# saidwivedi/TokenHMR

Measured on NVIDIA H100. Metric: images/sec (256x192) at bs=64 per GPU, full TokenHMR forward, higher is better.
Workload: dtype f16 operands / f32 accumulate

## Files before the change

tokenhmr_b200/csrc/attention_mma.cuh:

```cuda
#pragma once
#include "common.cuh"
#include "ptx.cuh"

namespace thmr {

constexpr int kAttTokens = 192;
constexpr int kAttHeadDim = 80;
constexpr int kAttPitch = 88;
constexpr int kAttWarps = 6;
constexpr int kAttThreads = 32 * kAttWarps;
constexpr uint32_t kAttMatBytes = kAttTokens * kAttPitch * 2;
constexpr uint32_t kAttSmemBytes = 3 * kAttMatBytes;

struct AttnParams {
  const __half* qkv;
  int ldq;
  int num_problems;
  int heads;
  float scale_log2e;
  __half* out;
  int ldo;
  float* dbg_s;
  unsigned long long* stamp;
};

__device__ __forceinline__ float fast_exp2(float x) {
  float y;
  asm("ex2.approx.ftz.f32 %0, %1;" : "=f"(y) : "f"(x));
  return y;
}
__device__ __forceinline__ void ldmatrix_x4(uint32_t (&r)[4], uint32_t addr) {
  asm volatile("ldmatrix.sync.aligned.m8n8.x4.shared.b16 {%0, %1, %2, %3}, [%4];"
               : "=r"(r[0]), "=r"(r[1]), "=r"(r[2]), "=r"(r[3]) : "r"(addr));
}
__device__ __forceinline__ void ldmatrix_x4_trans(uint32_t (&r)[4], uint32_t addr) {
  asm volatile("ldmatrix.sync.aligned.m8n8.x4.trans.shared.b16 {%0, %1, %2, %3}, [%4];"
               : "=r"(r[0]), "=r"(r[1]), "=r"(r[2]), "=r"(r[3]) : "r"(addr));
}
__device__ __forceinline__ void mma_16816(float (&d)[4], const uint32_t (&a)[4], uint32_t b0, uint32_t b1) {
  asm volatile("mma.sync.aligned.m16n8k16.row.col.f32.f16.f16.f32 {%0, %1, %2, %3}, {%4, %5, %6, %7}, {%8, %9}, "
               "{%0, %1, %2, %3};"
               : "+f"(d[0]), "+f"(d[1]), "+f"(d[2]), "+f"(d[3])
               : "r"(a[0]), "r"(a[1]), "r"(a[2]), "r"(a[3]), "r"(b0), "r"(b1));
}
__device__ __forceinline__ uint32_t pack_half2(float a, float b) {
  __half2 h = __floats2half2_rn(a, b);
  return *reinterpret_cast<uint32_t*>(&h);
}

template <bool DBG>
__global__ void __launch_bounds__(kAttThreads, 2) vit_attention_kernel(const AttnParams p) {
  extern __shared__ __align__(16) uint8_t att_smem[];
  const uint32_t aQ = smem_u32(att_smem), aK = aQ + kAttMatBytes, aV = aK + kAttMatBytes;
  const int prob = blockIdx.x;
  const int b = prob / p.heads, h = prob % p.heads;
  const int warp = threadIdx.x >> 5, lane = threadIdx.x & 31;

  pdl_launch_dependents();
  stamp_start(p.stamp);
  pdl_wait();

  const __half* src = p.qkv + static_cast<size_t>(b) * kAttTokens * p.ldq;
  for (int i = threadIdx.x; i < 3 * kAttTokens * 10; i += kAttThreads) {
    const int m = i / (kAttTokens * 10), r = (i / 10) % kAttTokens, c = i % 10;
    const __half* g = src + static_cast<size_t>(r) * p.ldq + (m * p.heads + h) * kAttHeadDim + c * 8;
    const uint32_t s = aQ + m * kAttMatBytes + (r * kAttPitch + c * 8) * 2;
    asm volatile("cp.async.cg.shared.global [%0], [%1], 16;" ::"r"(s), "l"(g) : "memory");
  }
  asm volatile("cp.async.commit_group;\n\tcp.async.wait_group 0;" ::: "memory");
  __syncthreads();

  const int g = lane >> 2, t4 = lane & 3;
  for (int tile = warp; tile < kAttTokens / 16; tile += kAttWarps) {
    const int r0 = tile * 16;
    uint32_t qa[5][4];
#pragma unroll
    for (int kk = 0; kk < 5; ++kk)
      ldmatrix_x4(qa[kk], aQ + ((r0 + (lane & 15)) * kAttPitch + kk * 16 + 8 * (lane >> 4)) * 2);
    float s[24][4];
#pragma unroll
    for (int nt = 0; nt < 24; ++nt) s[nt][0] = s[nt][1] = s[nt][2] = s[nt][3] = 0.f;
#pragma unroll
    for (int np = 0; np < 12; ++np) {
#pragma unroll
      for (int kk = 0; kk < 5; ++kk) {
        uint32_t kb[4];
        ldmatrix_x4(kb, aK + ((np * 16 + (lane & 7) + 8 * (lane >> 4)) * kAttPitch + kk * 16 + 8 * ((lane >> 3) & 1)) * 2);
        mma_16816(s[2 * np], qa[kk], kb[0], kb[1]);
        mma_16816(s[2 * np + 1], qa[kk], kb[2], kb[3]);
      }
    }
    if (DBG) {
      float* d = p.dbg_s + (static_cast<size_t>(prob) * kAttTokens + r0 + g) * kAttTokens + 2 * t4;
#pragma unroll
      for (int nt = 0; nt < 24; ++nt) {
        *reinterpret_cast<float2*>(d + nt * 8) = make_float2(s[nt][0], s[nt][1]);
        *reinterpret_cast<float2*>(d + 8 * kAttTokens + nt * 8) = make_float2(s[nt][2], s[nt][3]);
      }
    }
    float mx0 = -INFINITY, mx1 = -INFINITY;
#pragma unroll
    for (int nt = 0; nt < 24; ++nt) {
      mx0 = fmaxf(mx0, fmaxf(s[nt][0], s[nt][1]));
      mx1 = fmaxf(mx1, fmaxf(s[nt][2], s[nt][3]));
    }
#pragma unroll
    for (int off = 1; off <= 2; off <<= 1) {
      mx0 = fmaxf(mx0, __shfl_xor_sync(0xffffffffu, mx0, off));
      mx1 = fmaxf(mx1, __shfl_xor_sync(0xffffffffu, mx1, off));
    }
    const float mo0 = mx0 * p.scale_log2e, mo1 = mx1 * p.scale_log2e;
    float sum0 = 0.f, sum1 = 0.f;
    uint32_t pa[12][4];
#pragma unroll
    for (int nt = 0; nt < 24; ++nt) {
      const float e0 = fast_exp2(fmaf(s[nt][0], p.scale_log2e, -mo0));
      const float e1 = fast_exp2(fmaf(s[nt][1], p.scale_log2e, -mo0));
      const float e2 = fast_exp2(fmaf(s[nt][2], p.scale_log2e, -mo1));
      const float e3 = fast_exp2(fmaf(s[nt][3], p.scale_log2e, -mo1));
      sum0 += e0 + e1;
      sum1 += e2 + e3;
      pa[nt >> 1][(nt & 1) * 2 + 0] = pack_half2(e0, e1);
      pa[nt >> 1][(nt & 1) * 2 + 1] = pack_half2(e2, e3);
    }
#pragma unroll
    for (int off = 1; off <= 2; off <<= 1) {
      sum0 += __shfl_xor_sync(0xffffffffu, sum0, off);
      sum1 += __shfl_xor_sync(0xffffffffu, sum1, off);
    }
    float o[10][4];
#pragma unroll
    for (int dt = 0; dt < 10; ++dt) o[dt][0] = o[dt][1] = o[dt][2] = o[dt][3] = 0.f;
#pragma unroll
    for (int ks = 0; ks < 12; ++ks) {
#pragma unroll
      for (int dp = 0; dp < 5; ++dp) {
        uint32_t vb[4];
        ldmatrix_x4_trans(vb, aV + ((ks * 16 + (lane & 7) + 8 * ((lane >> 3) & 1)) * kAttPitch + dp * 16 + 8 * (lane >> 4)) * 2);
        mma_16816(o[2 * dp], pa[ks], vb[0], vb[1]);
        mma_16816(o[2 * dp + 1], pa[ks], vb[2], vb[3]);
      }
    }
    const float inv0 = 1.0f / sum0, inv1 = 1.0f / sum1;
    __half* out = p.out + (static_cast<size_t>(b) * kAttTokens + r0 + g) * p.ldo + h * kAttHeadDim + 2 * t4;
#pragma unroll
    for (int dt = 0; dt < 10; ++dt) {
      *reinterpret_cast<uint32_t*>(out + dt * 8) = pack_half2(o[dt][0] * inv0, o[dt][1] * inv0);
      *reinterpret_cast<uint32_t*>(out + 8 * static_cast<size_t>(p.ldo) + dt * 8) = pack_half2(o[dt][2] * inv1, o[dt][3] * inv1);
    }
  }
}

struct AttnPlan {
  AttnParams p;
  int grid;
};

inline int attention_make_plan(const __half* qkv, int ld_qkv, int B, int heads, __half* out, int ldo, float* dbg_s,
                               AttnPlan* plan) {
  THMR_CHECK(B > 0 && heads > 0, "attention: bad shape");
  THMR_CHECK(ld_qkv >= 3 * heads * kAttHeadDim, "attention: qkv pitch %d < %d", ld_qkv, 3 * heads * kAttHeadDim);
  THMR_CHECK((reinterpret_cast<uintptr_t>(qkv) & 15) == 0 && ld_qkv % 8 == 0, "attention: qkv pointer/pitch alignment");
  THMR_CHECK(ldo % 2 == 0 && (reinterpret_cast<uintptr_t>(out) & 3) == 0, "attention: output alignment");
  plan->p.qkv = qkv;
  plan->p.ldq = ld_qkv;
  plan->p.num_problems = B * heads;
  plan->p.heads = heads;
  plan->p.scale_log2e = 1.4426950408889634f / sqrtf(static_cast<float>(kAttHeadDim));
  plan->p.out = out;
  plan->p.ldo = ldo;
  plan->p.dbg_s = dbg_s;
  plan->p.stamp = nullptr;
  plan->grid = plan->p.num_problems;
  return THMR_OK;
}

template <bool DBG>
inline int attention_launch_t(const AttnPlan& plan, cudaStream_t st) {
  static bool configured = false;
  if (!configured) {
    THMR_CUDA(cudaFuncSetAttribute(vit_attention_kernel<DBG>, cudaFuncAttributeMaxDynamicSharedMemorySize, kAttSmemBytes));
    configured = true;
  }
  THMR_CUDA(launch_pdl(vit_attention_kernel<DBG>, plan.grid, kAttThreads, kAttSmemBytes, st, plan.p));
  return THMR_OK;
}

inline int attention_dispatch(const AttnPlan& plan, cudaStream_t st) {
  return plan.p.dbg_s ? attention_launch_t<true>(plan, st) : attention_launch_t<false>(plan, st);
}

}
```

tokenhmr_b200/_build.py:

```python
from __future__ import annotations

import hashlib
import os
import subprocess
import sys
from pathlib import Path

PKG_DIR = Path(__file__).resolve().parent
CSRC = PKG_DIR / "csrc"
LIB_PATH = PKG_DIR / "libtokenhmr_b200.so"
STAMP = PKG_DIR / ".libtokenhmr_b200.stamp"
PROBE_SRC = PKG_DIR.parent / "tests" / "csrc" / "kernel_probe.cu"
PROBE_PATH = PKG_DIR.parent / "tests" / "libthmr_probe.so"
PROBE_STAMP = PKG_DIR.parent / "tests" / ".libthmr_probe.stamp"
GEMM_PROBE_SRC = PKG_DIR.parent / "tests" / "csrc" / "gemm_probe.cu"
GEMM_PROBE_PATH = PKG_DIR.parent / "tests" / "libthmr_gemm_probe.so"
GEMM_PROBE_STAMP = PKG_DIR.parent / "tests" / ".libthmr_gemm_probe.stamp"

NVCC_FLAGS = [
    "-gencode", "arch=compute_90a,code=sm_90a",
    "-lineinfo", "-O3", "-std=c++17",
    "--expt-relaxed-constexpr",
    "-Xcompiler", "-fPIC", "-shared",
]
PROBE_FLAGS = ["-Xcompiler", "-fvisibility=hidden"]


def _nvcc() -> str:
    for cand in (os.environ.get("NVCC"), "/usr/local/cuda/bin/nvcc", "nvcc"):
        if cand and (os.path.isabs(cand) and os.path.exists(cand) or not os.path.isabs(cand)):
            return cand
    return "nvcc"


def source_hash(probe: bool = False) -> str:
    h = hashlib.sha256()
    files = sorted(CSRC.glob("*.cu")) + sorted(CSRC.glob("*.cuh")) + sorted((PKG_DIR.parent / "include").glob("*.h"))
    if probe:
        files += sorted(PROBE_SRC.parent.glob("*.cu"))
    for f in files:
        h.update(f.name.encode())
        h.update(f.read_bytes())
    h.update(" ".join(NVCC_FLAGS + (PROBE_FLAGS if probe else [])).encode())
    return h.hexdigest()


def _compile(src: Path, out: Path, stamp: Path, flags: list, want: str, force: bool, verbose: bool) -> Path:
    if not force and out.exists() and stamp.exists() and stamp.read_text().strip() == want:
        return out
    cmd = [_nvcc(), *flags, "-o", str(out), str(src)]
    if verbose:
        cmd.insert(1, "-Xptxas=-v")
        print(" ".join(cmd), file=sys.stderr)
    res = subprocess.run(cmd, capture_output=True, text=True)
    if res.returncode != 0:
        raise RuntimeError(f"nvcc failed ({res.returncode}):\n{res.stdout}\n{res.stderr}")
    if verbose:
        print(res.stderr, file=sys.stderr)
    stamp.write_text(want)
    return out


def build_probe(force: bool = False, verbose: bool = False) -> Path:
    if GEMM_PROBE_SRC.exists():
        _compile(GEMM_PROBE_SRC, GEMM_PROBE_PATH, GEMM_PROBE_STAMP, NVCC_FLAGS + PROBE_FLAGS, source_hash(probe=True),
                 force, verbose)
    return _compile(PROBE_SRC, PROBE_PATH, PROBE_STAMP, NVCC_FLAGS + PROBE_FLAGS, source_hash(probe=True), force,
                    verbose)


def build(force: bool = False, verbose: bool = False) -> Path:
    path = _compile(CSRC / "tokenhmr_b200.cu", LIB_PATH, STAMP, NVCC_FLAGS, source_hash(), force, verbose)
    if PROBE_SRC.exists():
        build_probe(force, verbose)
    return path


if __name__ == "__main__":
    print(build(force="--force" in sys.argv, verbose="-v" in sys.argv))
```

tokenhmr_b200/csrc/ptx.cuh:

```cuda
#pragma once
#include <cuda.h>
#include <cuda_fp16.h>
#include <cuda_runtime.h>
#include <stdint.h>

namespace thmr {

__device__ unsigned int g_pipeline_timeout = 0;
constexpr uint32_t kSpinLimit = 1u << 24;

__device__ __forceinline__ uint32_t smem_u32(const void* p) {
  return static_cast<uint32_t>(__cvta_generic_to_shared(p));
}

__device__ __forceinline__ void sts_f32x2(uint32_t a, float x, float y) {
  asm volatile("st.shared.v2.f32 [%0], {%1, %2};" ::"r"(a), "f"(x), "f"(y));
}
__device__ __forceinline__ float4 lds_f32x4(uint32_t a) {
  float4 v;
  asm volatile("ld.shared.v4.f32 {%0, %1, %2, %3}, [%4];" : "=f"(v.x), "=f"(v.y), "=f"(v.z), "=f"(v.w) : "r"(a));
  return v;
}
__device__ __forceinline__ void sts_f32(uint32_t a, float x) { asm volatile("st.shared.f32 [%0], %1;" ::"r"(a), "f"(x)); }
__device__ __forceinline__ void sts_u32(uint32_t a, uint32_t x) { asm volatile("st.shared.b32 [%0], %1;" ::"r"(a), "r"(x)); }
// ... 70 lines not shown
  asm volatile("barrier.cluster.arrive.release;\n\tbarrier.cluster.wait.acquire;" ::: "memory");
}
__device__ __forceinline__ void mbar_arrive_cluster(uint64_t* bar, uint32_t cta) {
  asm volatile(
      "{\n\t"
      ".reg .b32 ra;\n\t"
      "mapa.shared::cluster.u32 ra, %0, %1;\n\t"
      "mbarrier.arrive.release.cluster.shared::cluster.b64 _, [ra];\n\t"
      "}\n" ::"r"(smem_u32(bar)),
      "r"(cta)
      : "memory");
}
__device__ __forceinline__ bool mbar_wait_cluster(uint64_t* bar, uint32_t parity) {
#pragma unroll 1
  for (uint32_t it = 0; it < kSpinLimit; ++it) {
    uint32_t ok;
    asm volatile(
        "{\n\t"
        ".reg .pred P;\n\t"
        "mbarrier.try_wait.parity.acquire.cluster.shared::cta.b64 P, [%1], %2;\n\t"
        "selp.u32 %0, 1, 0, P;\n\t"
        "}\n"
        : "=r"(ok)
        : "r"(smem_u32(bar)), "r"(parity)
        : "memory");
    if (ok) return true;
  }
  atomicExch(&g_pipeline_timeout, 1u);
  return false;
}

__device__ __forceinline__ void tma_prefetch_desc(const CUtensorMap* m) {
  asm volatile("prefetch.tensormap [%0];" ::"l"(reinterpret_cast<uint64_t>(m)) : "memory");
}
__device__ __forceinline__ void tma_load_2d(void* smem_dst, const CUtensorMap* m, uint64_t* bar, int32_t c0,
                                            int32_t c1) {
  asm volatile(
      "cp.async.bulk.tensor.2d.shared::cluster.global.mbarrier::complete_tx::bytes"
      " [%0], [%1, {%3, %4}], [%2];"
      :
      : "r"(smem_u32(smem_dst)), "l"(reinterpret_cast<uint64_t>(m)), "r"(smem_u32(bar)), "r"(c0), "r"(c1)
      : "memory");
}
__device__ __forceinline__ void tma_load_2d_mcast(void* smem_dst, const CUtensorMap* m, uint64_t* bar, int32_t c0,
                                                  int32_t c1, uint16_t cta_mask) {
  asm volatile(
      "cp.async.bulk.tensor.2d.shared::cluster.global.mbarrier::complete_tx::bytes.multicast::cluster"
      " [%0], [%1, {%3, %4}], [%2], %5;"
      :
      : "r"(smem_u32(smem_dst)), "l"(reinterpret_cast<uint64_t>(m)), "r"(smem_u32(bar)), "r"(c0), "r"(c1),
        "h"(cta_mask)
      : "memory");
}
__device__ __forceinline__ void tma_store_2d(const CUtensorMap* m, uint32_t smem_src, int32_t c0, int32_t c1) {
  asm volatile("cp.async.bulk.tensor.2d.global.shared::cta.bulk_group [%0, {%2, %3}], [%1];"
               :
               : "l"(reinterpret_cast<uint64_t>(m)), "r"(smem_src), "r"(c0), "r"(c1)
               : "memory");
}
__device__ __forceinline__ void tma_reduce_add_2d(const CUtensorMap* m, uint32_t smem_src, int32_t c0, int32_t c1) {
  asm volatile("cp.reduce.async.bulk.tensor.2d.global.shared::cta.add.tile.bulk_group [%0, {%2, %3}], [%1];"
               :
               : "l"(reinterpret_cast<uint64_t>(m)), "r"(smem_src), "r"(c0), "r"(c1)
               : "memory");
}
__device__ __forceinline__ void tma_store_commit() { asm volatile("cp.async.bulk.commit_group;" ::: "memory"); }
template <int N>
__device__ __forceinline__ void tma_store_wait_read() {
  asm volatile("cp.async.bulk.wait_group.read %0;" ::"n"(N) : "memory");
}
template <int N>
__device__ __forceinline__ void tma_store_wait() {
  asm volatile("cp.async.bulk.wait_group %0;" ::"n"(N) : "memory");
}

__device__ __forceinline__ uint64_t make_wgmma_desc_sw128(uint32_t saddr) {
  uint64_t d = 0;
  d |= static_cast<uint64_t>((saddr >> 4) & 0x3FFF);
  d |= static_cast<uint64_t>(1) << 16;
  d |= static_cast<uint64_t>(1024 >> 4) << 32;
  d |= static_cast<uint64_t>(1) << 62;
  return d;
}
__device__ __forceinline__ void wgmma_fence() { asm volatile("wgmma.fence.sync.aligned;" ::: "memory"); }
__device__ __forceinline__ void wgmma_commit() { asm volatile("wgmma.commit_group.sync.aligned;" ::: "memory"); }
template <int N>
__device__ __forceinline__ void wgmma_wait() {
  asm volatile("wgmma.wait_group.sync.aligned %0;" ::"n"(N) : "memory");
}
template <int N>
__device__ __forceinline__ void wgmma_fence_operand(float (&d)[N]) {
#pragma unroll
  for (int i = 0; i < N; ++i) asm volatile("" : "+f"(d[i])::"memory");
}

__device__ __forceinline__ void wgmma_m64n32k16(float (&d)[16], uint64_t da, uint64_t db, uint32_t scale_d) {
  asm volatile(
      "{\n\t.reg .pred p;\n\tsetp.ne.b32 p, %18, 0;\n\t"
      "wgmma.mma_async.sync.aligned.m64n32k16.f32.f16.f16 {%0, %1, %2, %3, %4, %5, %6, %7, %8, %9, %10, %11, %12, %13, %14, %15}, %16, %17, p, 1, 1, 0, 0;\n\t}\n"
      : "+f"(d[0]), "+f"(d[1]), "+f"(d[2]), "+f"(d[3]), "+f"(d[4]), "+f"(d[5]), "+f"(d[6]), "+f"(d[7]), "+f"(d[8]), "+f"(d[9]), "+f"(d[10]), "+f"(d[11]), "+f"(d[12]), "+f"(d[13]), "+f"(d[14]), "+f"(d[15])
      : "l"(da), "l"(db), "r"(scale_d));
}
__device__ __forceinline__ void wgmma_m64n64k16(float (&d)[32], uint64_t da, uint64_t db, uint32_t scale_d) {
  asm volatile(
      "{\n\t.reg .pred p;\n\tsetp.ne.b32 p, %34, 0;\n\t"
      "wgmma.mma_async.sync.aligned.m64n64k16.f32.f16.f16 {%0, %1, %2, %3, %4, %5, %6, %7, %8, %9, %10, %11, %12, %13, %14, %15, %16, %17, %18, %19, %20, %21, %22, %23, %24, %25, %26, %27, %28, %29, %30, %31}, %32, %33, p, 1, 1, 0, 0;\n\t}\n"
      : "+f"(d[0]), "+f"(d[1]), "+f"(d[2]), "+f"(d[3]), "+f"(d[4]), "+f"(d[5]), "+f"(d[6]), "+f"(d[7]), "+f"(d[8]), "+f"(d[9]), "+f"(d[10]), "+f"(d[11]), "+f"(d[12]), "+f"(d[13]), "+f"(d[14]), "+f"(d[15]), "+f"(d[16]), "+f"(d[17]), "+f"(d[18]), "+f"(d[19]), "+f"(d[20]), "+f"(d[21]), "+f"(d[22]), "+f"(d[23]), "+f"(d[24]), "+f"(d[25]), "+f"(d[26]), "+f"(d[27]), "+f"(d[28]), "+f"(d[29]), "+f"(d[30]), "+f"(d[31])
      : "l"(da), "l"(db), "r"(scale_d));
}
__device__ __forceinline__ void wgmma_m64n128k16(float (&d)[64], uint64_t da, uint64_t db, uint32_t scale_d) {
  asm volatile(
      "{\n\t.reg .pred p;\n\tsetp.ne.b32 p, %66, 0;\n\t"
      "wgmma.mma_async.sync.aligned.m64n128k16.f32.f16.f16 {%0, %1, %2, %3, %4, %5, %6, %7, %8, %9, %10, %11, %12, %13, %14, %15, %16, %17, %18, %19, %20, %21, %22, %23, %24, %25, %26, %27, %28, %29, %30, %31, %32, %33, %34, %35, %36, %37, %38, %39, %40, %41, %42, %43, %44, %45, %46, %47, %48, %49, %50, %51, %52, %53, %54, %55, %56, %57, %58, %59, %60, %61, %62, %63}, %64, %65, p, 1, 1, 0, 0;\n\t}\n"
      : "+f"(d[0]), "+f"(d[1]), "+f"(d[2]), "+f"(d[3]), "+f"(d[4]), "+f"(d[5]), "+f"(d[6]), "+f"(d[7]), "+f"(d[8]), "+f"(d[9]), "+f"(d[10]), "+f"(d[11]), "+f"(d[12]), "+f"(d[13]), "+f"(d[14]), "+f"(d[15]), "+f"(d[16]), "+f"(d[17]), "+f"(d[18]), "+f"(d[19]), "+f"(d[20]), "+f"(d[21]), "+f"(d[22]), "+f"(d[23]), "+f"(d[24]), "+f"(d[25]), "+f"(d[26]), "+f"(d[27]), "+f"(d[28]), "+f"(d[29]), "+f"(d[30]), "+f"(d[31]), "+f"(d[32]), "+f"(d[33]), "+f"(d[34]), "+f"(d[35]), "+f"(d[36]), "+f"(d[37]), "+f"(d[38]), "+f"(d[39]), "+f"(d[40]), "+f"(d[41]), "+f"(d[42]), "+f"(d[43]), "+f"(d[44]), "+f"(d[45]), "+f"(d[46]), "+f"(d[47]), "+f"(d[48]), "+f"(d[49]), "+f"(d[50]), "+f"(d[51]), "+f"(d[52]), "+f"(d[53]), "+f"(d[54]), "+f"(d[55]), "+f"(d[56]), "+f"(d[57]), "+f"(d[58]), "+f"(d[59]), "+f"(d[60]), "+f"(d[61]), "+f"(d[62]), "+f"(d[63])
      : "l"(da), "l"(db), "r"(scale_d));
}
__device__ __forceinline__ void wgmma_m64n256k16(float (&d)[128], uint64_t da, uint64_t db, uint32_t scale_d) {
  asm volatile(
      "{\n\t.reg .pred p;\n\tsetp.ne.b32 p, %130, 0;\n\t"
      "wgmma.mma_async.sync.aligned.m64n256k16.f32.f16.f16 {%0, %1, %2, %3, %4, %5, %6, %7, %8, %9, %10, %11, %12, %13, %14, %15, %16, %17, %18, %19, %20, %21, %22, %23, %24, %25, %26, %27, %28, %29, %30, %31, %32, %33, %34, %35, %36, %37, %38, %39, %40, %41, %42, %43, %44, %45, %46, %47, %48, %49, %50, %51, %52, %53, %54, %55, %56, %57, %58, %59, %60, %61, %62, %63, %64, %65, %66, %67, %68, %69, %70, %71, %72, %73, %74, %75, %76, %77, %78, %79, %80, %81, %82, %83, %84, %85, %86, %87, %88, %89, %90, %91, %92, %93, %94, %95, %96, %97, %98, %99, %100, %101, %102, %103, %104, %105, %106, %107, %108, %109, %110, %111, %112, %113, %114, %115, %116, %117, %118, %119, %120, %121, %122, %123, %124, %125, %126, %127}, %128, %129, p, 1, 1, 0, 0;\n\t}\n"
      : "+f"(d[0]), "+f"(d[1]), "+f"(d[2]), "+f"(d[3]), "+f"(d[4]), "+f"(d[5]), "+f"(d[6]), "+f"(d[7]), "+f"(d[8]), "+f"(d[9]), "+f"(d[10]), "+f"(d[11]), "+f"(d[12]), "+f"(d[13]), "+f"(d[14]), "+f"(d[15]), "+f"(d[16]), "+f"(d[17]), "+f"(d[18]), "+f"(d[19]), "+f"(d[20]), "+f"(d[21]), "+f"(d[22]), "+f"(d[23]), "+f"(d[24]), "+f"(d[25]), "+f"(d[26]), "+f"(d[27]), "+f"(d[28]), "+f"(d[29]), "+f"(d[30]), "+f"(d[31]), "+f"(d[32]), "+f"(d[33]), "+f"(d[34]), "+f"(d[35]), "+f"(d[36]), "+f"(d[37]), "+f"(d[38]), "+f"(d[39]), "+f"(d[40]), "+f"(d[41]), "+f"(d[42]), "+f"(d[43]), "+f"(d[44]), "+f"(d[45]), "+f"(d[46]), "+f"(d[47]), "+f"(d[48]), "+f"(d[49]), "+f"(d[50]), "+f"(d[51]), "+f"(d[52]), "+f"(d[53]), "+f"(d[54]), "+f"(d[55]), "+f"(d[56]), "+f"(d[57]), "+f"(d[58]), "+f"(d[59]), "+f"(d[60]), "+f"(d[61]), "+f"(d[62]), "+f"(d[63]), "+f"(d[64]), "+f"(d[65]), "+f"(d[66]), "+f"(d[67]), "+f"(d[68]), "+f"(d[69]), "+f"(d[70]), "+f"(d[71]), "+f"(d[72]), "+f"(d[73]), "+f"(d[74]), "+f"(d[75]), "+f"(d[76]), "+f"(d[77]), "+f"(d[78]), "+f"(d[79]), "+f"(d[80]), "+f"(d[81]), "+f"(d[82]), "+f"(d[83]), "+f"(d[84]), "+f"(d[85]), "+f"(d[86]), "+f"(d[87]), "+f"(d[88]), "+f"(d[89]), "+f"(d[90]), "+f"(d[91]), "+f"(d[92]), "+f"(d[93]), "+f"(d[94]), "+f"(d[95]), "+f"(d[96]), "+f"(d[97]), "+f"(d[98]), "+f"(d[99]), "+f"(d[100]), "+f"(d[101]), "+f"(d[102]), "+f"(d[103]), "+f"(d[104]), "+f"(d[105]), "+f"(d[106]), "+f"(d[107]), "+f"(d[108]), "+f"(d[109]), "+f"(d[110]), "+f"(d[111]), "+f"(d[112]), "+f"(d[113]), "+f"(d[114]), "+f"(d[115]), "+f"(d[116]), "+f"(d[117]), "+f"(d[118]), "+f"(d[119]), "+f"(d[120]), "+f"(d[121]), "+f"(d[122]), "+f"(d[123]), "+f"(d[124]), "+f"(d[125]), "+f"(d[126]), "+f"(d[127])
      : "l"(da), "l"(db), "r"(scale_d));
}

__device__ __forceinline__ void wgmma_m64n64k32_e4m3(float (&d)[32], uint64_t da, uint64_t db, uint32_t scale_d) {
  asm volatile(
      "{\n\t.reg .pred p;\n\tsetp.ne.b32 p, %34, 0;\n\t"
      "wgmma.mma_async.sync.aligned.m64n64k32.f32.e4m3.e4m3 {%0, %1, %2, %3, %4, %5, %6, %7, %8, %9, %10, %11, %12, %13, %14, %15, %16, %17, %18, %19, %20, %21, %22, %23, %24, %25, %26, %27, %28, %29, %30, %31}, %32, %33, p, 1, 1;\n\t}\n"
      : "+f"(d[0]), "+f"(d[1]), "+f"(d[2]), "+f"(d[3]), "+f"(d[4]), "+f"(d[5]), "+f"(d[6]), "+f"(d[7]), "+f"(d[8]), "+f"(d[9]), "+f"(d[10]), "+f"(d[11]), "+f"(d[12]), "+f"(d[13]), "+f"(d[14]), "+f"(d[15]), "+f"(d[16]), "+f"(d[17]), "+f"(d[18]), "+f"(d[19]), "+f"(d[20]), "+f"(d[21]), "+f"(d[22]), "+f"(d[23]), "+f"(d[24]), "+f"(d[25]), "+f"(d[26]), "+f"(d[27]), "+f"(d[28]), "+f"(d[29]), "+f"(d[30]), "+f"(d[31])
      : "l"(da), "l"(db), "r"(scale_d));
}
__device__ __forceinline__ void wgmma_m64n128k32_e4m3(float (&d)[64], uint64_t da, uint64_t db, uint32_t scale_d) {
  asm volatile(
      "{\n\t.reg .pred p;\n\tsetp.ne.b32 p, %66, 0;\n\t"
      "wgmma.mma_async.sync.aligned.m64n128k32.f32.e4m3.e4m3 {%0, %1, %2, %3, %4, %5, %6, %7, %8, %9, %10, %11, %12, %13, %14, %15, %16, %17, %18, %19, %20, %21, %22, %23, %24, %25, %26, %27, %28, %29, %30, %31, %32, %33, %34, %35, %36, %37, %38, %39, %40, %41, %42, %43, %44, %45, %46, %47, %48, %49, %50, %51, %52, %53, %54, %55, %56, %57, %58, %59, %60, %61, %62, %63}, %64, %65, p, 1, 1;\n\t}\n"
      : "+f"(d[0]), "+f"(d[1]), "+f"(d[2]), "+f"(d[3]), "+f"(d[4]), "+f"(d[5]), "+f"(d[6]), "+f"(d[7]), "+f"(d[8]), "+f"(d[9]), "+f"(d[10]), "+f"(d[11]), "+f"(d[12]), "+f"(d[13]), "+f"(d[14]), "+f"(d[15]), "+f"(d[16]), "+f"(d[17]), "+f"(d[18]), "+f"(d[19]), "+f"(d[20]), "+f"(d[21]), "+f"(d[22]), "+f"(d[23]), "+f"(d[24]), "+f"(d[25]), "+f"(d[26]), "+f"(d[27]), "+f"(d[28]), "+f"(d[29]), "+f"(d[30]), "+f"(d[31]), "+f"(d[32]), "+f"(d[33]), "+f"(d[34]), "+f"(d[35]), "+f"(d[36]), "+f"(d[37]), "+f"(d[38]), "+f"(d[39]), "+f"(d[40]), "+f"(d[41]), "+f"(d[42]), "+f"(d[43]), "+f"(d[44]), "+f"(d[45]), "+f"(d[46]), "+f"(d[47]), "+f"(d[48]), "+f"(d[49]), "+f"(d[50]), "+f"(d[51]), "+f"(d[52]), "+f"(d[53]), "+f"(d[54]), "+f"(d[55]), "+f"(d[56]), "+f"(d[57]), "+f"(d[58]), "+f"(d[59]), "+f"(d[60]), "+f"(d[61]), "+f"(d[62]), "+f"(d[63])
      : "l"(da), "l"(db), "r"(scale_d));
}

__device__ __forceinline__ uint16_t cvt_e4m3x2(float lo, float hi) {
  uint16_t r;
  asm("cvt.rn.satfinite.e4m3x2.f32 %0, %1, %2;" : "=h"(r) : "f"(hi), "f"(lo));
  return r;
}

__device__ __forceinline__ float e4m3_scale(float amax) {
  if (!(amax > 0.f)) return 1.0f;
  int E;
  const float m = frexpf(amax, &E);
  return ldexpf(1.0f, m <= 0.875f ? E - 9 : E - 8);
}

__device__ __forceinline__ void bulk_load_1d(void* smem_dst, const void* src, uint32_t bytes, uint64_t* bar) {
  asm volatile("cp.async.bulk.shared::cluster.global.mbarrier::complete_tx::bytes [%0], [%1], %2, [%3];"
               :
               : "r"(smem_u32(smem_dst)), "l"(reinterpret_cast<uint64_t>(src)), "r"(bytes), "r"(smem_u32(bar))
               : "memory");
}

}
```

Baseline: 1901.

## Make ViT attention persistent with double-buffered TMA loads and staged output stores

The attention kernel now runs as a persistent grid sized to the SM count, with 12 warps per CTA so that each warp owns one 16-row query tile. Q/K/V for each (batch, head) problem are fetched with 2D TMA into one of two shared-memory buffers guarded by mbarriers, so the next problem's load overlaps the current problem's compute. This replaces the per-thread cp.async loop and its full wait. Output tiles are first written into the warp's own Q rows in shared memory and then stored to global as coalesced 16-byte chunks, which tightens the output alignment requirements. The CTA now uses about twice the shared memory and runs at one CTA per SM instead of two.

```diff
diff --git a/tokenhmr_b200/csrc/attention_mma.cuh b/tokenhmr_b200/csrc/attention_mma.cuh
--- a/tokenhmr_b200/csrc/attention_mma.cuh
+++ b/tokenhmr_b200/csrc/attention_mma.cuh
@@ -7,14 +7,14 @@
 constexpr int kAttTokens = 192;
 constexpr int kAttHeadDim = 80;
 constexpr int kAttPitch = 88;
-constexpr int kAttWarps = 6;
+constexpr int kAttWarps = kAttTokens / 16;
 constexpr int kAttThreads = 32 * kAttWarps;
 constexpr uint32_t kAttMatBytes = kAttTokens * kAttPitch * 2;
-constexpr uint32_t kAttSmemBytes = 3 * kAttMatBytes;
+constexpr uint32_t kAttBufBytes = 3 * kAttMatBytes;
+constexpr uint32_t kAttSmemBytes = 2 * kAttBufBytes + 2 * sizeof(uint64_t);
 
 struct AttnParams {
-  const __half* qkv;
-  int ldq;
+  CUtensorMap tm_qkv;
   int num_problems;
   int heads;
   float scale_log2e;
@@ -48,31 +48,44 @@
   return *reinterpret_cast<uint32_t*>(&h);
 }
 
+__device__ __forceinline__ void attention_load(const AttnParams& p, uint8_t* buf, uint64_t* bar, int prob) {
+  const int b = prob / p.heads, h = prob % p.heads;
+  mbar_arrive_expect_tx(bar, kAttBufBytes);
+#pragma unroll
+  for (int m = 0; m < 3; ++m)
+    tma_load_2d(buf + m * kAttMatBytes, &p.tm_qkv, bar, (m * p.heads + h) * kAttHeadDim, b * kAttTokens);
+}
+
 template <bool DBG>
-__global__ void __launch_bounds__(kAttThreads, 2) vit_attention_kernel(const AttnParams p) {
-  extern __shared__ __align__(16) uint8_t att_smem[];
-  const uint32_t aQ = smem_u32(att_smem), aK = aQ + kAttMatBytes, aV = aK + kAttMatBytes;
-  const int prob = blockIdx.x;
-  const int b = prob / p.heads, h = prob % p.heads;
+__global__ void __launch_bounds__(kAttThreads, 1) vit_attention_kernel(const __grid_constant__ AttnParams p) {
+  extern __shared__ __align__(128) uint8_t att_smem[];
+  uint64_t* full = reinterpret_cast<uint64_t*>(att_smem + 2 * kAttBufBytes);
   const int warp = threadIdx.x >> 5, lane = threadIdx.x & 31;
+  const int n = p.num_problems;
 
   pdl_launch_dependents();
   stamp_start(p.stamp);
+  if (threadIdx.x == 0) {
+    tma_prefetch_desc(&p.tm_qkv);
+    mbar_init(&full[0], 1);
+    mbar_init(&full[1], 1);
+    fence_mbar_init();
+  }
+  __syncthreads();
   pdl_wait();
 
-  const __half* src = p.qkv + static_cast<size_t>(b) * kAttTokens * p.ldq;
-  for (int i = threadIdx.x; i < 3 * kAttTokens * 10; i += kAttThreads) {
-    const int m = i / (kAttTokens * 10), r = (i / 10) % kAttTokens, c = i % 10;
-    const __half* g = src + static_cast<size_t>(r) * p.ldq + (m * p.heads + h) * kAttHeadDim + c * 8;
-    const uint32_t s = aQ + m * kAttMatBytes + (r * kAttPitch + c * 8) * 2;
-    asm volatile("cp.async.cg.shared.global [%0], [%1], 16;" ::"r"(s), "l"(g) : "memory");
-  }
-  asm volatile("cp.async.commit_group;\n\tcp.async.wait_group 0;" ::: "memory");
-  __syncthreads();
-
+  if (threadIdx.x == 0) attention_load(p, att_smem, &full[0], n - 1 - static_cast<int>(blockIdx.x));
   const int g = lane >> 2, t4 = lane & 3;
-  for (int tile = warp; tile < kAttTokens / 16; tile += kAttWarps) {
-    const int r0 = tile * 16;
+  const int r0 = warp * 16;
+  for (int it = 0, idx = blockIdx.x; idx < n; ++it, idx += gridDim.x) {
+    const int buf = it & 1;
+    const int next = idx + gridDim.x;
+    if (threadIdx.x == 0 && next < n) attention_load(p, att_smem + (buf ^ 1) * kAttBufBytes, &full[buf ^ 1], n - 1 - next);
+    const int prob = n - 1 - idx;
+    const int b = prob / p.heads, h = prob % p.heads;
+    const uint32_t aQ = smem_u32(att_smem) + buf * kAttBufBytes, aK = aQ + kAttMatBytes, aV = aK + kAttMatBytes;
+    mbar_wait(&full[buf], (it >> 1) & 1);
+
     uint32_t qa[5][4];
 #pragma unroll
     for (int kk = 0; kk < 5; ++kk)
@@ -142,12 +155,22 @@
       }
     }
     const float inv0 = 1.0f / sum0, inv1 = 1.0f / sum1;
-    __half* out = p.out + (static_cast<size_t>(b) * kAttTokens + r0 + g) * p.ldo + h * kAttHeadDim + 2 * t4;
+    const uint32_t stage = aQ + r0 * kAttPitch * 2;
+    __syncwarp();
 #pragma unroll
     for (int dt = 0; dt < 10; ++dt) {
-      *reinterpret_cast<uint32_t*>(out + dt * 8) = pack_half2(o[dt][0] * inv0, o[dt][1] * inv0);
-      *reinterpret_cast<uint32_t*>(out + 8 * static_cast<size_t>(p.ldo) + dt * 8) = pack_half2(o[dt][2] * inv1, o[dt][3] * inv1);
-    }
+      sts_u32(stage + (g * kAttPitch + dt * 8 + 2 * t4) * 2, pack_half2(o[dt][0] * inv0, o[dt][1] * inv0));
+      sts_u32(stage + ((g + 8) * kAttPitch + dt * 8 + 2 * t4) * 2, pack_half2(o[dt][2] * inv1, o[dt][3] * inv1));
+    }
+    __syncwarp();
+    __half* out = p.out + (static_cast<size_t>(b) * kAttTokens + r0) * p.ldo + h * kAttHeadDim;
+#pragma unroll 1
+    for (int c = lane; c < 16 * kAttHeadDim / 8; c += 32) {
+      const int r = c / (kAttHeadDim / 8), c8 = c % (kAttHeadDim / 8);
+      *reinterpret_cast<float4*>(out + static_cast<size_t>(r) * p.ldo + c8 * 8) = lds_f32x4(stage + (r * kAttPitch + c8 * 8) * 2);
+    }
+    fence_proxy_async_smem();
+    __syncthreads();
   }
 }
 
@@ -161,9 +184,10 @@
   THMR_CHECK(B > 0 && heads > 0, "attention: bad shape");
   THMR_CHECK(ld_qkv >= 3 * heads * kAttHeadDim, "attention: qkv pitch %d < %d", ld_qkv, 3 * heads * kAttHeadDim);
   THMR_CHECK((reinterpret_cast<uintptr_t>(qkv) & 15) == 0 && ld_qkv % 8 == 0, "attention: qkv pointer/pitch alignment");
-  THMR_CHECK(ldo % 2 == 0 && (reinterpret_cast<uintptr_t>(out) & 3) == 0, "attention: output alignment");
-  plan->p.qkv = qkv;
-  plan->p.ldq = ld_qkv;
+  THMR_CHECK(ldo >= heads * kAttHeadDim && ldo % 8 == 0 && (reinterpret_cast<uintptr_t>(out) & 15) == 0,
+             "attention: output pitch %d / pointer alignment (16-byte row pieces)", ldo);
+  THMR_TRY(make_tmap_2d_f16(&plan->p.tm_qkv, qkv, static_cast<uint64_t>(B) * kAttTokens, 3ull * heads * kAttHeadDim,
+                            ld_qkv, kAttTokens, kAttPitch, CU_TENSOR_MAP_SWIZZLE_NONE));
   plan->p.num_problems = B * heads;
   plan->p.heads = heads;
   plan->p.scale_log2e = 1.4426950408889634f / sqrtf(static_cast<float>(kAttHeadDim));
@@ -171,7 +195,7 @@
   plan->p.ldo = ldo;
   plan->p.dbg_s = dbg_s;
   plan->p.stamp = nullptr;
-  plan->grid = plan->p.num_problems;
+  plan->grid = plan->p.num_problems < num_sms() ? plan->p.num_problems : num_sms();
   return THMR_OK;
 }
 
```

Measured after the change: 1923 (median of 6 runs). No clear change (+1.2%).

## Rewrite ViT attention as persistent warp-specialized TMA+WGMMA kernel

Applied to the files above, without the earlier changes.

Replaces the per-head mma.sync attention kernel, which loaded with cp.async and used ldmatrix, with a persistent kernel. One producer warp issues TMA loads of Q, K and V into swizzled shared memory with a two-stage mbarrier pipeline. Three consumer warpgroups each compute a 64-row tile of QK^T with m64n192 wgmma and P·V with register-sourced wgmma. The intent is to cut load latency and instruction overhead and to overlap the next head's loads with current compute. The costs are lower occupancy (one block per SM), extra tensor-map setup, and reliance on correct swizzle descriptors for the 80-wide head dim split into 64+16 boxes.

```diff
diff --git a/tokenhmr_b200/_build.py b/tokenhmr_b200/_build.py
--- a/tokenhmr_b200/_build.py
+++ b/tokenhmr_b200/_build.py
@@ -16,6 +16,9 @@
 GEMM_PROBE_SRC = PKG_DIR.parent / "tests" / "csrc" / "gemm_probe.cu"
 GEMM_PROBE_PATH = PKG_DIR.parent / "tests" / "libthmr_gemm_probe.so"
 GEMM_PROBE_STAMP = PKG_DIR.parent / "tests" / ".libthmr_gemm_probe.stamp"
+ATTN_PROBE_SRC = PKG_DIR.parent / "tests" / "csrc" / "attention_probe.cu"
+ATTN_PROBE_PATH = PKG_DIR.parent / "tests" / "libthmr_attention_probe.so"
+ATTN_PROBE_STAMP = PKG_DIR.parent / "tests" / ".libthmr_attention_probe.stamp"
 
 NVCC_FLAGS = [
     "-gencode", "arch=compute_90a,code=sm_90a",
@@ -62,9 +65,10 @@
 
 
 def build_probe(force: bool = False, verbose: bool = False) -> Path:
-    if GEMM_PROBE_SRC.exists():
-        _compile(GEMM_PROBE_SRC, GEMM_PROBE_PATH, GEMM_PROBE_STAMP, NVCC_FLAGS + PROBE_FLAGS, source_hash(probe=True),
-                 force, verbose)
+    for src, out, stamp in ((GEMM_PROBE_SRC, GEMM_PROBE_PATH, GEMM_PROBE_STAMP),
+                            (ATTN_PROBE_SRC, ATTN_PROBE_PATH, ATTN_PROBE_STAMP)):
+        if src.exists():
+            _compile(src, out, stamp, NVCC_FLAGS + PROBE_FLAGS, source_hash(probe=True), force, verbose)
     return _compile(PROBE_SRC, PROBE_PATH, PROBE_STAMP, NVCC_FLAGS + PROBE_FLAGS, source_hash(probe=True), force,
                     verbose)
 
diff --git a/tokenhmr_b200/csrc/attention_mma.cuh b/tokenhmr_b200/csrc/attention_mma.cuh
--- a/tokenhmr_b200/csrc/attention_mma.cuh
+++ b/tokenhmr_b200/csrc/attention_mma.cuh
@@ -6,13 +6,21 @@
 
 constexpr int kAttTokens = 192;
 constexpr int kAttHeadDim = 80;
-constexpr int kAttPitch = 88;
-constexpr int kAttWarps = 6;
-constexpr int kAttThreads = 32 * kAttWarps;
-constexpr uint32_t kAttMatBytes = kAttTokens * kAttPitch * 2;
-constexpr uint32_t kAttSmemBytes = 3 * kAttMatBytes;
+constexpr int kAttConsumerWGs = 3;
+constexpr int kAttThreads = 128 * (kAttConsumerWGs + 1);
+constexpr int kAttStages = 2;
+constexpr uint32_t kAttBox64Bytes = kAttTokens * 128;
+constexpr uint32_t kAttBox16Bytes = kAttTokens * 32;
+constexpr uint32_t kAttMatBytes = kAttBox64Bytes + kAttBox16Bytes;
+constexpr uint32_t kAttStageBytes = 3 * kAttMatBytes;
+constexpr uint32_t kAttBarOffset = kAttStages * kAttStageBytes;
+constexpr uint32_t kAttSmemBytes = kAttBarOffset + 3 * kAttStages * 8 + 1024;
+static_assert(kAttConsumerWGs * 64 == kAttTokens, "one 64-row wgmma tile per consumer warpgroup");
+static_assert(kAttBox64Bytes % 1024 == 0 && kAttMatBytes % 1024 == 0, "128B-swizzled boxes need 1024-B alignment");
 
 struct AttnParams {
+  CUtensorMap tm64;
+  CUtensorMap tm16;
   const __half* qkv;
   int ldq;
   int num_problems;
@@ -29,80 +37,99 @@
   asm("ex2.approx.ftz.f32 %0, %1;" : "=f"(y) : "f"(x));
   return y;
 }
-__device__ __forceinline__ void ldmatrix_x4(uint32_t (&r)[4], uint32_t addr) {
-  asm volatile("ldmatrix.sync.aligned.m8n8.x4.shared.b16 {%0, %1, %2, %3}, [%4];"
-               : "=r"(r[0]), "=r"(r[1]), "=r"(r[2]), "=r"(r[3]) : "r"(addr));
-}
-__device__ __forceinline__ void ldmatrix_x4_trans(uint32_t (&r)[4], uint32_t addr) {
-  asm volatile("ldmatrix.sync.aligned.m8n8.x4.trans.shared.b16 {%0, %1, %2, %3}, [%4];"
-               : "=r"(r[0]), "=r"(r[1]), "=r"(r[2]), "=r"(r[3]) : "r"(addr));
-}
-__device__ __forceinline__ void mma_16816(float (&d)[4], const uint32_t (&a)[4], uint32_t b0, uint32_t b1) {
-  asm volatile("mma.sync.aligned.m16n8k16.row.col.f32.f16.f16.f32 {%0, %1, %2, %3}, {%4, %5, %6, %7}, {%8, %9}, "
-               "{%0, %1, %2, %3};"
-               : "+f"(d[0]), "+f"(d[1]), "+f"(d[2]), "+f"(d[3])
-               : "r"(a[0]), "r"(a[1]), "r"(a[2]), "r"(a[3]), "r"(b0), "r"(b1));
-}
 __device__ __forceinline__ uint32_t pack_half2(float a, float b) {
   __half2 h = __floats2half2_rn(a, b);
   return *reinterpret_cast<uint32_t*>(&h);
 }
+__device__ __forceinline__ void attn_item(const AttnParams& p, int i, int& b, int& h) {
+  b = p.num_problems / p.heads - 1 - i / p.heads;
+  h = i % p.heads;
+}
 
 template <bool DBG>
-__global__ void __launch_bounds__(kAttThreads, 2) vit_attention_kernel(const AttnParams p) {
-  extern __shared__ __align__(16) uint8_t att_smem[];
-  const uint32_t aQ = smem_u32(att_smem), aK = aQ + kAttMatBytes, aV = aK + kAttMatBytes;
-  const int prob = blockIdx.x;
-  const int b = prob / p.heads, h = prob % p.heads;
+__global__ void __launch_bounds__(kAttThreads, 1) vit_attention_kernel(const __grid_constant__ AttnParams p) {
+  extern __shared__ uint8_t att_smem_raw[];
+  uint8_t* smem = reinterpret_cast<uint8_t*>((reinterpret_cast<uintptr_t>(att_smem_raw) + 1023) & ~uintptr_t(1023));
+  uint64_t* full_qk = reinterpret_cast<uint64_t*>(smem + kAttBarOffset);
+  uint64_t* full_v = full_qk + kAttStages;
+  uint64_t* empty = full_v + kAttStages;
   const int warp = threadIdx.x >> 5, lane = threadIdx.x & 31;
+  const int wg = warp >> 2;
 
   pdl_launch_dependents();
   stamp_start(p.stamp);
+  if (threadIdx.x == 0) {
+    for (int s = 0; s < kAttStages; ++s) {
+      mbar_init(&full_qk[s], 1);
+      mbar_init(&full_v[s], 1);
+      mbar_init(&empty[s], kAttConsumerWGs);
+    }
+    fence_mbar_init();
+  }
+  __syncthreads();
   pdl_wait();
 
-  const __half* src = p.qkv + static_cast<size_t>(b) * kAttTokens * p.ldq;
-  for (int i = threadIdx.x; i < 3 * kAttTokens * 10; i += kAttThreads) {
-    const int m = i / (kAttTokens * 10), r = (i / 10) % kAttTokens, c = i % 10;
-    const __half* g = src + static_cast<size_t>(r) * p.ldq + (m * p.heads + h) * kAttHeadDim + c * 8;
-    const uint32_t s = aQ + m * kAttMatBytes + (r * kAttPitch + c * 8) * 2;
-    asm volatile("cp.async.cg.shared.global [%0], [%1], 16;" ::"r"(s), "l"(g) : "memory");
-  }
-  asm volatile("cp.async.commit_group;\n\tcp.async.wait_group 0;" ::: "memory");
-  __syncthreads();
-
+  if (wg == kAttConsumerWGs) {
+    asm volatile("setmaxnreg.dec.sync.aligned.u32 40;");
+    if (warp == 4 * kAttConsumerWGs && lane == 0) {
+      tma_prefetch_desc(&p.tm64);
+      tma_prefetch_desc(&p.tm16);
+      int stage = 0;
+      uint32_t phase = 0;
+      for (int i = blockIdx.x; i < p.num_problems; i += gridDim.x) {
+        int b, h;
+        attn_item(p, i, b, h);
+        mbar_wait(&empty[stage], phase ^ 1);
+        uint8_t* st = smem + stage * kAttStageBytes;
+        for (int m = 0; m < 3; ++m) {
+          uint64_t* bar = m < 2 ? &full_qk[stage] : &full_v[stage];
+          if (m != 1) mbar_arrive_expect_tx(bar, (m < 2 ? 2 : 1) * kAttMatBytes);
+          const int col = (m * p.heads + h) * kAttHeadDim;
+          tma_load_2d(st + m * kAttMatBytes, &p.tm64, bar, col, b * kAttTokens);
+          tma_load_2d(st + m * kAttMatBytes + kAttBox64Bytes, &p.tm16, bar, col + 64, b * kAttTokens);
+        }
+        if (++stage == kAttStages) { stage = 0; phase ^= 1; }
+      }
+    }
+    return;
+  }
+
+  asm volatile("setmaxnreg.inc.sync.aligned.u32 152;");
   const int g = lane >> 2, t4 = lane & 3;
-  for (int tile = warp; tile < kAttTokens / 16; tile += kAttWarps) {
-    const int r0 = tile * 16;
-    uint32_t qa[5][4];
-#pragma unroll
-    for (int kk = 0; kk < 5; ++kk)
-      ldmatrix_x4(qa[kk], aQ + ((r0 + (lane & 15)) * kAttPitch + kk * 16 + 8 * (lane >> 4)) * 2);
-    float s[24][4];
-#pragma unroll
-    for (int nt = 0; nt < 24; ++nt) s[nt][0] = s[nt][1] = s[nt][2] = s[nt][3] = 0.f;
-#pragma unroll
-    for (int np = 0; np < 12; ++np) {
-#pragma unroll
-      for (int kk = 0; kk < 5; ++kk) {
-        uint32_t kb[4];
-        ldmatrix_x4(kb, aK + ((np * 16 + (lane & 7) + 8 * (lane >> 4)) * kAttPitch + kk * 16 + 8 * ((lane >> 3) & 1)) * 2);
-        mma_16816(s[2 * np], qa[kk], kb[0], kb[1]);
-        mma_16816(s[2 * np + 1], qa[kk], kb[2], kb[3]);
+  const int r = wg * 64 + (warp & 3) * 16 + g;
+  const uint32_t base = smem_u32(smem);
+  int stage = 0;
+  uint32_t phase = 0;
+  for (int i = blockIdx.x; i < p.num_problems; i += gridDim.x) {
+    int b, h;
+    attn_item(p, i, b, h);
+    const uint32_t sQ = base + stage * kAttStageBytes, sK = sQ + kAttMatBytes, sV = sK + kAttMatBytes;
+
+    float s[96];
+    mbar_wait(&full_qk[stage], phase);
+    wgmma_fence();
+#pragma unroll
+    for (int kk = 0; kk < 4; ++kk)
+      wgmma_m64n192k16(s, make_wgmma_desc_sw128(sQ + wg * 64 * 128 + 32 * kk), make_wgmma_desc_sw128(sK + 32 * kk),
+                       kk > 0);
+    wgmma_m64n192k16(s, make_wgmma_desc_sw32(sQ + kAttBox64Bytes + wg * 64 * 32), make_wgmma_desc_sw32(sK + kAttBox64Bytes),
+                     1);
+    wgmma_commit();
+    wgmma_wait<0>();
+    wgmma_fence_operand(s);
+    if (DBG) {
+      float* d = p.dbg_s + ((static_cast<size_t>(b) * p.heads + h) * kAttTokens + r) * kAttTokens + 2 * t4;
+#pragma unroll
+      for (int nt = 0; nt < 24; ++nt) {
+        *reinterpret_cast<float2*>(d + nt * 8) = make_float2(s[4 * nt], s[4 * nt + 1]);
+        *reinterpret_cast<float2*>(d + 8 * kAttTokens + nt * 8) = make_float2(s[4 * nt + 2], s[4 * nt + 3]);
       }
     }
-    if (DBG) {
-      float* d = p.dbg_s + (static_cast<size_t>(prob) * kAttTokens + r0 + g) * kAttTokens + 2 * t4;
-#pragma unroll
-      for (int nt = 0; nt < 24; ++nt) {
-        *reinterpret_cast<float2*>(d + nt * 8) = make_float2(s[nt][0], s[nt][1]);
-        *reinterpret_cast<float2*>(d + 8 * kAttTokens + nt * 8) = make_float2(s[nt][2], s[nt][3]);
-      }
-    }
     float mx0 = -INFINITY, mx1 = -INFINITY;
 #pragma unroll
     for (int nt = 0; nt < 24; ++nt) {
-      mx0 = fmaxf(mx0, fmaxf(s[nt][0], s[nt][1]));
-      mx1 = fmaxf(mx1, fmaxf(s[nt][2], s[nt][3]));
+      mx0 = fmaxf(mx0, fmaxf(s[4 * nt], s[4 * nt + 1]));
+      mx1 = fmaxf(mx1, fmaxf(s[4 * nt + 2], s[4 * nt + 3]));
     }
 #pragma unroll
     for (int off = 1; off <= 2; off <<= 1) {
@@ -114,10 +141,10 @@
     uint32_t pa[12][4];
 #pragma unroll
     for (int nt = 0; nt < 24; ++nt) {
-      const float e0 = fast_exp2(fmaf(s[nt][0], p.scale_log2e, -mo0));
-      const float e1 = fast_exp2(fmaf(s[nt][1], p.scale_log2e, -mo0));
-      const float e2 = fast_exp2(fmaf(s[nt][2], p.scale_log2e, -mo1));
-      const float e3 = fast_exp2(fmaf(s[nt][3], p.scale_log2e, -mo1));
+      const float e0 = fast_exp2(fmaf(s[4 * nt], p.scale_log2e, -mo0));
+      const float e1 = fast_exp2(fmaf(s[4 * nt + 1], p.scale_log2e, -mo0));
+      const float e2 = fast_exp2(fmaf(s[4 * nt + 2], p.scale_log2e, -mo1));
+      const float e3 = fast_exp2(fmaf(s[4 * nt + 3], p.scale_log2e, -mo1));
       sum0 += e0 + e1;
       sum1 += e2 + e3;
       pa[nt >> 1][(nt & 1) * 2 + 0] = pack_half2(e0, e1);
@@ -128,25 +155,29 @@
       sum0 += __shfl_xor_sync(0xffffffffu, sum0, off);
       sum1 += __shfl_xor_sync(0xffffffffu, sum1, off);
     }
-    float o[10][4];
-#pragma unroll
-    for (int dt = 0; dt < 10; ++dt) o[dt][0] = o[dt][1] = o[dt][2] = o[dt][3] = 0.f;
+
+    float o64[32], o16[8];
+    mbar_wait(&full_v[stage], phase);
+    wgmma_fence();
 #pragma unroll
     for (int ks = 0; ks < 12; ++ks) {
-#pragma unroll
-      for (int dp = 0; dp < 5; ++dp) {
-        uint32_t vb[4];
-        ldmatrix_x4_trans(vb, aV + ((ks * 16 + (lane & 7) + 8 * ((lane >> 3) & 1)) * kAttPitch + dp * 16 + 8 * (lane >> 4)) * 2);
-        mma_16816(o[2 * dp], pa[ks], vb[0], vb[1]);
-        mma_16816(o[2 * dp + 1], pa[ks], vb[2], vb[3]);
-      }
-    }
+      wgmma_m64n64k16_rs_tb(o64, pa[ks], make_wgmma_desc_sw128(sV + ks * 16 * 128), ks > 0);
+      wgmma_m64n16k16_rs_tb(o16, pa[ks], make_wgmma_desc_sw32(sV + kAttBox64Bytes + ks * 16 * 32), ks > 0);
+    }
+    wgmma_commit();
+    wgmma_wait<0>();
+    wgmma_fence_operand(o64);
+    wgmma_fence_operand(o16);
+    if ((threadIdx.x & 127) == 0) mbar_arrive(&empty[stage]);
+    if (++stage == kAttStages) { stage = 0; phase ^= 1; }
+
     const float inv0 = 1.0f / sum0, inv1 = 1.0f / sum1;
-    __half* out = p.out + (static_cast<size_t>(b) * kAttTokens + r0 + g) * p.ldo + h * kAttHeadDim + 2 * t4;
+    __half* out = p.out + (static_cast<size_t>(b) * kAttTokens + r) * p.ldo + h * kAttHeadDim + 2 * t4;
 #pragma unroll
     for (int dt = 0; dt < 10; ++dt) {
-      *reinterpret_cast<uint32_t*>(out + dt * 8) = pack_half2(o[dt][0] * inv0, o[dt][1] * inv0);
-      *reinterpret_cast<uint32_t*>(out + 8 * static_cast<size_t>(p.ldo) + dt * 8) = pack_half2(o[dt][2] * inv1, o[dt][3] * inv1);
+      const float* o = dt < 8 ? o64 + 4 * dt : o16 + 4 * (dt - 8);
+      *reinterpret_cast<uint32_t*>(out + dt * 8) = pack_half2(o[0] * inv0, o[1] * inv0);
+      *reinterpret_cast<uint32_t*>(out + 8 * static_cast<size_t>(p.ldo) + dt * 8) = pack_half2(o[2] * inv1, o[3] * inv1);
     }
   }
 }
@@ -162,6 +193,9 @@
   THMR_CHECK(ld_qkv >= 3 * heads * kAttHeadDim, "attention: qkv pitch %d < %d", ld_qkv, 3 * heads * kAttHeadDim);
   THMR_CHECK((reinterpret_cast<uintptr_t>(qkv) & 15) == 0 && ld_qkv % 8 == 0, "attention: qkv pointer/pitch alignment");
   THMR_CHECK(ldo % 2 == 0 && (reinterpret_cast<uintptr_t>(out) & 3) == 0, "attention: output alignment");
+  const uint64_t rows = static_cast<uint64_t>(B) * kAttTokens, cols = 3 * heads * kAttHeadDim;
+  THMR_TRY(make_tmap_2d_f16(&plan->p.tm64, qkv, rows, cols, ld_qkv, kAttTokens, 64, CU_TENSOR_MAP_SWIZZLE_128B));
+  THMR_TRY(make_tmap_2d_f16(&plan->p.tm16, qkv, rows, cols, ld_qkv, kAttTokens, 16, CU_TENSOR_MAP_SWIZZLE_32B));
   plan->p.qkv = qkv;
   plan->p.ldq = ld_qkv;
   plan->p.num_problems = B * heads;
@@ -171,7 +205,7 @@
   plan->p.ldo = ldo;
   plan->p.dbg_s = dbg_s;
   plan->p.stamp = nullptr;
-  plan->grid = plan->p.num_problems;
+  plan->grid = plan->p.num_problems < num_sms() ? plan->p.num_problems : num_sms();
   return THMR_OK;
 }
 
diff --git a/tokenhmr_b200/csrc/ptx.cuh b/tokenhmr_b200/csrc/ptx.cuh
--- a/tokenhmr_b200/csrc/ptx.cuh
+++ b/tokenhmr_b200/csrc/ptx.cuh
@@ -176,6 +176,14 @@
   d |= static_cast<uint64_t>(1) << 62;
   return d;
 }
+__device__ __forceinline__ uint64_t make_wgmma_desc_sw32(uint32_t saddr) {
+  uint64_t d = 0;
+  d |= static_cast<uint64_t>((saddr >> 4) & 0x3FFF);
+  d |= static_cast<uint64_t>(1) << 16;
+  d |= static_cast<uint64_t>(256 >> 4) << 32;
+  d |= static_cast<uint64_t>(3) << 62;
+  return d;
+}
 __device__ __forceinline__ void wgmma_fence() { asm volatile("wgmma.fence.sync.aligned;" ::: "memory"); }
 __device__ __forceinline__ void wgmma_commit() { asm volatile("wgmma.commit_group.sync.aligned;" ::: "memory"); }
 template <int N>
@@ -215,6 +223,29 @@
       "wgmma.mma_async.sync.aligned.m64n256k16.f32.f16.f16 {%0, %1, %2, %3, %4, %5, %6, %7, %8, %9, %10, %11, %12, %13, %14, %15, %16, %17, %18, %19, %20, %21, %22, %23, %24, %25, %26, %27, %28, %29, %30, %31, %32, %33, %34, %35, %36, %37, %38, %39, %40, %41, %42, %43, %44, %45, %46, %47, %48, %49, %50, %51, %52, %53, %54, %55, %56, %57, %58, %59, %60, %61, %62, %63, %64, %65, %66, %67, %68, %69, %70, %71, %72, %73, %74, %75, %76, %77, %78, %79, %80, %81, %82, %83, %84, %85, %86, %87, %88, %89, %90, %91, %92, %93, %94, %95, %96, %97, %98, %99, %100, %101, %102, %103, %104, %105, %106, %107, %108, %109, %110, %111, %112, %113, %114, %115, %116, %117, %118, %119, %120, %121, %122, %123, %124, %125, %126, %127}, %128, %129, p, 1, 1, 0, 0;\n\t}\n"
       : "+f"(d[0]), "+f"(d[1]), "+f"(d[2]), "+f"(d[3]), "+f"(d[4]), "+f"(d[5]), "+f"(d[6]), "+f"(d[7]), "+f"(d[8]), "+f"(d[9]), "+f"(d[10]), "+f"(d[11]), "+f"(d[12]), "+f"(d[13]), "+f"(d[14]), "+f"(d[15]), "+f"(d[16]), "+f"(d[17]), "+f"(d[18]), "+f"(d[19]), "+f"(d[20]), "+f"(d[21]), "+f"(d[22]), "+f"(d[23]), "+f"(d[24]), "+f"(d[25]), "+f"(d[26]), "+f"(d[27]), "+f"(d[28]), "+f"(d[29]), "+f"(d[30]), "+f"(d[31]), "+f"(d[32]), "+f"(d[33]), "+f"(d[34]), "+f"(d[35]), "+f"(d[36]), "+f"(d[37]), "+f"(d[38]), "+f"(d[39]), "+f"(d[40]), "+f"(d[41]), "+f"(d[42]), "+f"(d[43]), "+f"(d[44]), "+f"(d[45]), "+f"(d[46]), "+f"(d[47]), "+f"(d[48]), "+f"(d[49]), "+f"(d[50]), "+f"(d[51]), "+f"(d[52]), "+f"(d[53]), "+f"(d[54]), "+f"(d[55]), "+f"(d[56]), "+f"(d[57]), "+f"(d[58]), "+f"(d[59]), "+f"(d[60]), "+f"(d[61]), "+f"(d[62]), "+f"(d[63]), "+f"(d[64]), "+f"(d[65]), "+f"(d[66]), "+f"(d[67]), "+f"(d[68]), "+f"(d[69]), "+f"(d[70]), "+f"(d[71]), "+f"(d[72]), "+f"(d[73]), "+f"(d[74]), "+f"(d[75]), "+f"(d[76]), "+f"(d[77]), "+f"(d[78]), "+f"(d[79]), "+f"(d[80]), "+f"(d[81]), "+f"(d[82]), "+f"(d[83]), "+f"(d[84]), "+f"(d[85]), "+f"(d[86]), "+f"(d[87]), "+f"(d[88]), "+f"(d[89]), "+f"(d[90]), "+f"(d[91]), "+f"(d[92]), "+f"(d[93]), "+f"(d[94]), "+f"(d[95]), "+f"(d[96]), "+f"(d[97]), "+f"(d[98]), "+f"(d[99]), "+f"(d[100]), "+f"(d[101]), "+f"(d[102]), "+f"(d[103]), "+f"(d[104]), "+f"(d[105]), "+f"(d[106]), "+f"(d[107]), "+f"(d[108]), "+f"(d[109]), "+f"(d[110]), "+f"(d[111]), "+f"(d[112]), "+f"(d[113]), "+f"(d[114]), "+f"(d[115]), "+f"(d[116]), "+f"(d[117]), "+f"(d[118]), "+f"(d[119]), "+f"(d[120]), "+f"(d[121]), "+f"(d[122]), "+f"(d[123]), "+f"(d[124]), "+f"(d[125]), "+f"(d[126]), "+f"(d[127])
       : "l"(da), "l"(db), "r"(scale_d));
+}
+
+__device__ __forceinline__ void wgmma_m64n192k16(float (&d)[96], uint64_t da, uint64_t db, uint32_t scale_d) {
+  asm volatile(
+      "{\n\t.reg .pred p;\n\tsetp.ne.b32 p, %98, 0;\n\t"
+      "wgmma.mma_async.sync.aligned.m64n192k16.f32.f16.f16 {%0, %1, %2, %3, %4, %5, %6, %7, %8, %9, %10, %11, %12, %13, %14, %15, %16, %17, %18, %19, %20, %21, %22, %23, %24, %25, %26, %27, %28, %29, %30, %31, %32, %33, %34, %35, %36, %37, %38, %39, %40, %41, %42, %43, %44, %45, %46, %47, %48, %49, %50, %51, %52, %53, %54, %55, %56, %57, %58, %59, %60, %61, %62, %63, %64, %65, %66, %67, %68, %69, %70, %71, %72, %73, %74, %75, %76, %77, %78, %79, %80, %81, %82, %83, %84, %85, %86, %87, %88, %89, %90, %91, %92, %93, %94, %95}, %96, %97, p, 1, 1, 0, 0;\n\t}\n"
+      : "+f"(d[0]), "+f"(d[1]), "+f"(d[2]), "+f"(d[3]), "+f"(d[4]), "+f"(d[5]), "+f"(d[6]), "+f"(d[7]), "+f"(d[8]), "+f"(d[9]), "+f"(d[10]), "+f"(d[11]), "+f"(d[12]), "+f"(d[13]), "+f"(d[14]), "+f"(d[15]), "+f"(d[16]), "+f"(d[17]), "+f"(d[18]), "+f"(d[19]), "+f"(d[20]), "+f"(d[21]), "+f"(d[22]), "+f"(d[23]), "+f"(d[24]), "+f"(d[25]), "+f"(d[26]), "+f"(d[27]), "+f"(d[28]), "+f"(d[29]), "+f"(d[30]), "+f"(d[31]), "+f"(d[32]), "+f"(d[33]), "+f"(d[34]), "+f"(d[35]), "+f"(d[36]), "+f"(d[37]), "+f"(d[38]), "+f"(d[39]), "+f"(d[40]), "+f"(d[41]), "+f"(d[42]), "+f"(d[43]), "+f"(d[44]), "+f"(d[45]), "+f"(d[46]), "+f"(d[47]), "+f"(d[48]), "+f"(d[49]), "+f"(d[50]), "+f"(d[51]), "+f"(d[52]), "+f"(d[53]), "+f"(d[54]), "+f"(d[55]), "+f"(d[56]), "+f"(d[57]), "+f"(d[58]), "+f"(d[59]), "+f"(d[60]), "+f"(d[61]), "+f"(d[62]), "+f"(d[63]), "+f"(d[64]), "+f"(d[65]), "+f"(d[66]), "+f"(d[67]), "+f"(d[68]), "+f"(d[69]), "+f"(d[70]), "+f"(d[71]), "+f"(d[72]), "+f"(d[73]), "+f"(d[74]), "+f"(d[75]), "+f"(d[76]), "+f"(d[77]), "+f"(d[78]), "+f"(d[79]), "+f"(d[80]), "+f"(d[81]), "+f"(d[82]), "+f"(d[83]), "+f"(d[84]), "+f"(d[85]), "+f"(d[86]), "+f"(d[87]), "+f"(d[88]), "+f"(d[89]), "+f"(d[90]), "+f"(d[91]), "+f"(d[92]), "+f"(d[93]), "+f"(d[94]), "+f"(d[95])
+      : "l"(da), "l"(db), "r"(scale_d));
+}
+
+__device__ __forceinline__ void wgmma_m64n64k16_rs_tb(float (&d)[32], const uint32_t (&a)[4], uint64_t db, uint32_t scale_d) {
+  asm volatile(
+      "{\n\t.reg .pred p;\n\tsetp.ne.b32 p, %37, 0;\n\t"
+      "wgmma.mma_async.sync.aligned.m64n64k16.f32.f16.f16 {%0, %1, %2, %3, %4, %5, %6, %7, %8, %9, %10, %11, %12, %13, %14, %15, %16, %17, %18, %19, %20, %21, %22, %23, %24, %25, %26, %27, %28, %29, %30, %31}, {%32, %33, %34, %35}, %36, p, 1, 1, 1;\n\t}\n"
+      : "+f"(d[0]), "+f"(d[1]), "+f"(d[2]), "+f"(d[3]), "+f"(d[4]), "+f"(d[5]), "+f"(d[6]), "+f"(d[7]), "+f"(d[8]), "+f"(d[9]), "+f"(d[10]), "+f"(d[11]), "+f"(d[12]), "+f"(d[13]), "+f"(d[14]), "+f"(d[15]), "+f"(d[16]), "+f"(d[17]), "+f"(d[18]), "+f"(d[19]), "+f"(d[20]), "+f"(d[21]), "+f"(d[22]), "+f"(d[23]), "+f"(d[24]), "+f"(d[25]), "+f"(d[26]), "+f"(d[27]), "+f"(d[28]), "+f"(d[29]), "+f"(d[30]), "+f"(d[31])
+      : "r"(a[0]), "r"(a[1]), "r"(a[2]), "r"(a[3]), "l"(db), "r"(scale_d));
+}
+__device__ __forceinline__ void wgmma_m64n16k16_rs_tb(float (&d)[8], const uint32_t (&a)[4], uint64_t db, uint32_t scale_d) {
+  asm volatile(
+      "{\n\t.reg .pred p;\n\tsetp.ne.b32 p, %13, 0;\n\t"
+      "wgmma.mma_async.sync.aligned.m64n16k16.f32.f16.f16 {%0, %1, %2, %3, %4, %5, %6, %7}, {%8, %9, %10, %11}, %12, p, 1, 1, 1;\n\t}\n"
+      : "+f"(d[0]), "+f"(d[1]), "+f"(d[2]), "+f"(d[3]), "+f"(d[4]), "+f"(d[5]), "+f"(d[6]), "+f"(d[7])
+      : "r"(a[0]), "r"(a[1]), "r"(a[2]), "r"(a[3]), "l"(db), "r"(scale_d));
 }
 
 __device__ __forceinline__ void wgmma_m64n64k32_e4m3(float (&d)[32], uint64_t da, uint64_t db, uint32_t scale_d) {
```

Result: no change. 1891 before, 1921 after, median of 6 (+1.6%).
